# mycorrhiza-inc/fugu

Hardware: AMD Instinct MI355X
Metric: queries/sec + p50 latency, 10M-doc Zipf corpus, 3-term AND, top-100 (higher is better)
Workload: dtype u32+f32; 1 GPU; 3-term AND, BM25 top-100, 10M-doc Zipf s=1.0 corpus per namespace, batch 1024; n_docs=10000000, vocab=1048576, batch=1024, k=100, terms=3, namespaces=1, parallelism=namespace-shard x1

## Files before the change

fugu_amd/csrc/fg_host.h:

```cpp
#pragma once
#include <hip/hip_runtime.h>

#include <algorithm>
#include <atomic>
#include <chrono>
#include <condition_variable>
#include <functional>
#include <cstdint>
#include <map>
#include <memory>
#include <mutex>
#include <string>
#include <thread>
#include <vector>

#include "../../include/fugu.h"
#include "fg_internal.h"
#include "fg_pool.h"
#include "fg_trace.h"

namespace fgh {

int fail(int code, const char* fmt, ...);
int hw_threads(int req);
// ... 312 lines not shown
  std::shared_ptr<DevAllocs> smem;
  std::shared_ptr<ScorePool> spool;
  uint64_t struct_bytes = 0;
  fg::DevIndex d{};
};

struct IndexBounds {
  std::shared_ptr<ScoreBlock> sblock;
  const float* ktop = nullptr;
  const float* tmaxs = nullptr;
  SharedVec<float> wb_text, wb_name;
  float cache_b[512];
  SharedVec<uint32_t> h_alive_b;
  SharedVec<uint64_t> dtab_map;
  uint64_t dtab_bytes = 0;
  SharedVec<uint64_t> dtab8_map;
  uint64_t dtab8_bytes = 0;
  uint64_t device_bytes = 0;
};

inline uint32_t doctab_lead() {
  const char* e = getenv("FUGU_DOCTAB_LEAD");
  return e && *e ? (uint32_t)std::max(0l, atol(e)) : fg::kDocTabLead;
}

inline uint32_t doctab_slot(const IndexBounds& b, uint32_t t) {
  const auto it = std::lower_bound(b.dtab_map.begin(), b.dtab_map.end(), (uint64_t)t << 32);
  return it != b.dtab_map.end() && (uint32_t)(*it >> 32) == t ? (uint32_t)*it + 1u : 0u;
}

inline uint32_t doctab8_lead() {
  const char* e = getenv("FUGU_DOCTAB8_LEAD");
  return e && *e ? (uint32_t)std::max(0l, atol(e)) : fg::kDocTab8Lead;
}

inline uint32_t doctab8_slot(const IndexBounds& b, uint32_t t) {
  const auto it = std::lower_bound(b.dtab8_map.begin(), b.dtab8_map.end(), (uint64_t)t << 32);
  return it != b.dtab8_map.end() && (uint32_t)(*it >> 32) == t ? (uint32_t)*it + 1u : 0u;
}
}

struct fg_index : fgh::IndexStructure, fgh::IndexBounds {
  std::atomic<int> refs{1};
  int dev = 0;
  uint32_t n_dense = 0;
  uint64_t tot[2] = {0, 0};
  uint64_t n_stats = 0;
  float avgdl[2] = {0, 0};
  float cache[512];
  fgh::SharedVec<float> w_text, w_name;
  fgh::SharedVec<float> idf_text, idf_name;
  uint64_t tot_f = 0;
  float avgdl_f = 0.0f, cache_f1 = 0.0f;
  std::vector<uint32_t> df_facet;
  std::vector<float> fscore;
  fgh::SharedVec<uint32_t> h_alive;
  uint32_t n_dead = 0;
  bool same_stats = true;
  double cup[2] = {1, 1}, cdn[2] = {1, 1};
  std::shared_ptr<void> alive_hold;
  std::shared_ptr<const std::vector<float>> kth_floor;
  DevAllocs mem;
  std::shared_ptr<WsPool> pool;
  std::shared_ptr<PinnedPool> pinned;
};

// ... 21 lines not shown
  uint32_t n_prof = 0;
  ~fg_plan() {
    for (hipEvent_t e : pending) (void)hipEventDestroy(e);
    if (pin) {
      (void)hipSetDevice(ix->dev);
      (void)hipStreamSynchronize(up_stream);
    }
    if (ws) {
      if (last_stream_used) {
        (void)hipSetDevice(ix->dev);
        (void)hipStreamSynchronize(last_stream);
      }
      if (pin) ix->pinned->put(pin, pin_n);
      ix->pool->put(ws, ws_got);
    }
    if (!ipc_maps.empty()) {
      (void)hipSetDevice(ix->dev);
      for (void* m : ipc_maps) (void)hipIpcCloseMemHandle(m);
    }
    if (ix) fg_index_release(ix);
    for (fg_index* x : segs) fg_index_release(x);
  }
  bool last_stream_used = false;
  std::vector<uint32_t> h_lo, h_hi;
  std::vector<uint8_t> h_any;
  double part_next = 0.0;
  bool zeroed = false;
  void* pin = nullptr;
  size_t pin_n = 0;
  std::vector<void*> ipc_maps;
  hipStream_t up_stream = hipStreamPerThread;
};


namespace fgh {
inline uint32_t local_term(const fg_index* ix, uint32_t t) {
  if (ix->tmap.empty()) return t;
  const auto it = std::lower_bound(ix->tmap.begin(), ix->tmap.end(), t);
  return it != ix->tmap.end() && *it == t ? (uint32_t)(it - ix->tmap.begin()) : 0xFFFFFFFFu;
}
void term_ratio(const fg_index* ix, uint32_t t, float* rdn, float* rup);
float term_max_now(const fg_index* ix, uint32_t t);
float term_max_scaled(const fg_index* ix, uint32_t t, float rup);
float term_kth_now(const fg_index* ix, uint32_t t, uint32_t k, bool with_floor);

struct Bins { uint32_t lo, hi, shift; };
Bins union_bins(uint32_t lo, uint32_t hi);
int plan_create_multi(fg_index* const* ixs, uint32_t n_segs, const fg_query_batch* q, uint32_t k, fg_plan** out,
                      bool sync, hipStream_t up);
void run_parallel(uint32_t n, const std::function<void(uint32_t)>& f);

hipStream_t build_stream();
bool on_background();
uint32_t bg_grid_cap(int dev);
uint8_t fieldnorm_id(uint64_t n);
void bm25_weights(uint64_t Ns, const uint32_t* df_t, const uint32_t* df_n, uint32_t V, std::vector<float>& wt,
                  std::vector<float>& wn, std::vector<float>& it, std::vector<float>& in);
void set_stats(fg_index* ix, uint64_t Ns, const uint64_t tot2[2], const uint32_t* df_t, const uint32_t* df_n,
               uint64_t tot_f, const uint32_t* df_f, const Weights* wts);
void relate_stats(fg_index* ix);
int dev_upload_bytes(DevAllocs& m, const void* src, size_t n, void** out, uint64_t* bytes);
template <class T>
int dev_upload(DevAllocs& m, const T* src, size_t n, T** out, uint64_t* bytes) {
  return dev_upload_bytes(m, src, n * sizeof(T), reinterpret_cast<void**>(out), bytes);
}
struct UploadBatch {
// ... 20 lines not shown
```

fugu_amd/csrc/fg_internal.h:

```cpp
#pragma once
#include <algorithm>
#include <cstdint>
#include <initializer_list>

#include <hip/hip_runtime.h>

namespace fg {

constexpr uint32_t kBlock = 128;
#ifndef FG_BUCKET
#define FG_BUCKET 4
#endif
constexpr uint32_t kBucketTarget = FG_BUCKET;
constexpr uint32_t kThreads = 256;
#ifndef FG_ITEMS
#define FG_ITEMS 8
#endif
constexpr uint32_t kItems = FG_ITEMS;
constexpr uint32_t kChunk = kThreads * kItems;
constexpr uint32_t kWaveSpan = kChunk / 4;
constexpr uint32_t kMaxTerms = 16;
constexpr uint32_t kMaxK = 1024;
#ifndef FG_FINALCAP
#define FG_FINALCAP 4096
// ... 66 lines not shown
#ifndef FG_DISJ_ROUND
#define FG_DISJ_ROUND 512
#endif
#ifndef FG_DISJ_HBITS
#define FG_DISJ_HBITS 9
#endif
#ifndef FG_DISJ_WAVES
#define FG_DISJ_WAVES 5
#endif
#ifndef FG_DISJ_G
#define FG_DISJ_G 1
#endif
#ifndef FG_DISJ_MAXGROUP
#define FG_DISJ_MAXGROUP 32
#endif
constexpr uint32_t kDisjMaxGroup = FG_DISJ_MAXGROUP;
constexpr uint32_t kDisjMaxPairs = 256;
constexpr uint32_t kNumTopK = 5;
constexpr uint32_t kTopKs[kNumTopK] = {1, 10, 20, 100, 1000};
constexpr uint32_t kNumLadderExtra = 9;
constexpr uint32_t kLadderExtra[kNumLadderExtra] = {2, 3, 5, 13, 25, 50, 125, 250, 500};
constexpr uint32_t kNumLadder = kNumTopK + kNumLadderExtra;
constexpr uint32_t kLadderKs[kNumLadder] = {1, 2, 3, 5, 10, 13, 20, 25, 50, 100, 125, 250, 500, 1000};

constexpr uint32_t kPhraseMaxGroup = 4;
constexpr uint32_t kMaxFacetClauses = 8;
constexpr uint32_t kFmaskChunk = 8192;
constexpr uint32_t kScanMaxGroup = 32;

constexpr uint32_t kModeAnd = 0;
constexpr uint32_t kModeOr = 1;

constexpr uint32_t kQBins = 512;

__host__ __device__ inline uint32_t qm_terms(uint32_t qm) { return qm & 0xFFu; }
__host__ __device__ inline uint32_t qm_must(uint32_t qm) { return (qm >> 8) & 0xFFu; }
__host__ __device__ inline uint32_t qm_not(uint32_t qm) { return (qm >> 16) & 0xFFu; }
__host__ __device__ inline uint32_t qm_pack(uint32_t m, uint32_t nm, uint32_t nx) { return m | (nm << 8) | (nx << 16); }
__host__ __device__ inline uint32_t qm_phrase(uint32_t distinct, uint32_t n) { return distinct | (n << 24); }
__host__ __device__ inline uint32_t qm_phrase_terms(uint32_t qm) { return qm >> 24; }

__host__ __device__ inline uint32_t rank_word(uint32_t d) { return d >> 5; }
__host__ __device__ inline uint32_t rank_pos(uint64_t x, uint32_t d) {
#if defined(__HIP_DEVICE_COMPILE__)
  asm volatile("" : "+v"(d));
#endif
  const uint32_t b = d & 31u;
  if (!((x >> b) & 1ull)) return 0xFFFFFFFFu;
  const uint32_t below = (uint32_t)x & ((1u << b) - 1u);
#if defined(__HIP_DEVICE_COMPILE__)
  return (uint32_t)(x >> 32) + (uint32_t)__popc(below);
#else
  return (uint32_t)(x >> 32) + (uint32_t)__builtin_popcount(below);
#endif
}

__host__ __device__ inline uint32_t srank_block(uint32_t d) { return d >> 10; }
__host__ __device__ inline uint32_t srank_index(uint64_t e, uint32_t d) {
#if defined(__HIP_DEVICE_COMPILE__)
  asm volatile("" : "+v"(d));
#endif
  const uint32_t w = (d >> 5) & 31u;
  const uint32_t below = (uint32_t)e & ((1u << w) - 1u);
#if defined(__HIP_DEVICE_COMPILE__)
  const uint32_t i = (uint32_t)(e >> 32) + (uint32_t)__popc(below);
#else
// ... 176 lines not shown
  if (p1.kind & (kPdDir | kPdWide)) return false;
  if (!probe_uses_bound(ix.n_docs, df, lead_df, tab8_lead)) return false;
  const uint64_t a = (uint64_t)(uintptr_t)(ix.dtab8 + (uint64_t)(tab8 - 1) * ix.dtab8_stride);
  p1.aux_lo = (uint32_t)a;
  p1.kind = (p1.kind & 0xFFFFu) | kPdBound | (uint32_t)((a >> 32) & 0xFFFFu) << 16;
  union { float f; uint32_t u; } c;
  c.f = M;
  lead.aux_lo = c.u;
  return true;
}

struct DevFilters {
  uint32_t n_filters;
  uint32_t n_chunks;
  const uint32_t* q_filter;
  const uint32_t* f_shift;
  const uint64_t* f_woff;
  const float* f_tab;
  const float* f_max;
  const uint32_t* ch_filter;
  const uint32_t* ch_clause;
  const uint32_t* ch_term;
  const uint32_t* ch_start;
  const uint32_t* f_seg;
  uint32_t* fmask;
};

__host__ __device__ inline uint32_t filter_bits(const uint32_t* mask, uint32_t shift, uint32_t d) {
  const uint32_t bit = d << shift;
  return (mask[bit >> 5] >> (bit & 31)) & ((1u << (1u << shift)) - 1u);
}

constexpr uint32_t kMaxPeers = 15;

struct DevPlan {
  uint32_t n_queries;
  uint32_t total_chunks;
  uint32_t k;
  uint32_t n_conj;
  const uint32_t* q_m;
  const uint32_t* q_terms;
  const uint32_t* q_lead_df;
  const uint32_t* work_q;
  const uint32_t* work_c;
  const uint32_t* work_n;
  const uint64_t* cand_off;
  const uint64_t* q_thr0;
  const float* q_ub;
  const ProbeDesc* q_probe;
  const float* q_wt;
  const float* q_wn;
  const float* q_rup;
  const uint32_t* q_hlo;
  const uint32_t* q_hsh;
  uint64_t* thresh;
  uint32_t* hist;
  uint64_t pub_mask;
  uint32_t* cand_cnt;
  uint64_t* cand_keys;
  uint64_t* diag;
  uint32_t feat;
  uint32_t n_single;
  uint32_t n_scan;
  uint32_t n_phrase;
  const uint32_t* q_pterm;
  const uint32_t* q_ppos;
  const DevIndex* segs;
  uint32_t seg_nq;
  uint32_t n_segs;
  const uint32_t* seg_base;
  DevFilters f;
  uint32_t n_peers;
  uint32_t* peer_hist[kMaxPeers];
  uint64_t* peer_thr[kMaxPeers];
};

__host__ __device__ inline uint32_t slot_query(const DevPlan& pl, uint32_t v) {
  return pl.seg_nq ? v % pl.seg_nq : v;
}

constexpr uint32_t kCountItems = 8;
constexpr uint32_t kCountChunk = kThreads * kCountItems;
constexpr uint32_t kCountFacetChunk = kFmaskChunk;
constexpr uint32_t kCountFacetItems = kCountFacetChunk / kThreads;
constexpr uint32_t kCountWordChunk = 2048;
constexpr uint32_t kCountTile = 64;
constexpr uint32_t kCountText = 0, kCountFacet = 1, kCountFill = 2;
struct DevCount {
  uint32_t nq;
  uint32_t q0;
  uint32_t words;
  uint32_t n_count;
  uint32_t n_fchunks, n_items, n_cchunks;
  uint32_t* match;
// ... 169 lines not shown
```

fugu_amd/csrc/fugu.cpp:

```cpp
#include <hip/hip_runtime.h>
#include <sched.h>

#include <algorithm>
#include <atomic>
#include <chrono>
#include <cmath>
#include <condition_variable>
#include <deque>
#include <functional>
#include <cstdarg>
#include <cstdio>
#include <cstring>
#include <map>
#include <memory>
#include <mutex>
#include <string>
#include <thread>
#include <vector>

#include "../../include/fugu.h"
#include "fg_host.h"
#include "fg_internal.h"

namespace {
// ... 963 lines not shown
  return FG_OK;
}

int fg_plan_kernel_ms(fg_plan* p, double* ms_out, uint32_t* n_out) {
  if (!p) return fail(FG_EINVAL, "NULL plan");
  HIPCHK(hipSetDevice(p->ix->dev));
  for (size_t i = 0; i + 2 < p->pending.size(); i += 3) {
    HIPCHK(hipEventSynchronize(p->pending[i + 2]));
    for (int kx = 0; kx < 2; ++kx) {
      float ms = 0;
      HIPCHK(hipEventElapsedTime(&ms, p->pending[i + kx], p->pending[i + kx + 1]));
      p->ms[kx] += ms;
    }
    p->n_prof++;
  }
  for (hipEvent_t e : p->pending) (void)hipEventDestroy(e);
  p->pending.clear();
  if (ms_out) for (int kx = 0; kx < 2; ++kx) ms_out[kx] = p->ms[kx];
  if (n_out) *n_out = p->n_prof;
  p->ms[0] = p->ms[1] = 0;
  p->n_prof = 0;
  return FG_OK;
}

int fg_plan_diag(fg_plan* p, uint64_t* out, size_t n_words, uint32_t* cand_cnt) {
  if (!p) return fail(FG_EINVAL, "NULL plan");
  HIPCHK(hipSetDevice(p->ix->dev));
  HIPCHK(hipStreamSynchronize(p->last_stream));
  if (cand_cnt) HIPCHK(hipMemcpy(cand_cnt, p->d.cand_cnt, 4ull * p->nq, hipMemcpyDeviceToHost));
  if (out && n_words) {
    if (!p->d.diag) return fail(FG_EUNSUPPORTED, "not a diagnostic build (-DFG_DIAG)");
    HIPCHK(hipMemcpy(out, p->d.diag, 8 * std::min(n_words, p->diag_words), hipMemcpyDeviceToHost));
  }
  return FG_OK;
}

int fg_plan_destroy(fg_plan* p) {
  delete p;
  return FG_OK;
}

int fg_plan_link(fg_plan* const* plans, uint32_t n) {
  if (!plans || n == 0) return fail(FG_EINVAL, "bad arguments");
  fg_plan* o = plans[0];
  for (uint32_t i = 0; i < n; ++i) {
    if (!plans[i]) return fail(FG_EINVAL, "NULL plan");
    if (plans[i]->nq != o->nq || plans[i]->k != o->k) return fail(FG_EINVAL, "linked plans differ in batch or k");
    if (plans[i]->ix->dev != o->ix->dev) return fail(FG_EINVAL, "linked plans live on different devices");
    if (plans[i]->n_segs > 1) return fail(FG_EUNSUPPORTED, "a multi-snapshot plan already shares its thresholds");
  }
  const uint32_t nq = o->nq;
  std::vector<uint32_t> lo(nq, 0), sh(nq, 0);
  for (uint32_t q = 0; q < nq; ++q) {
    uint32_t l = 0, h = 0;
    for (uint32_t i = 0; i < n; ++i) {
      l = std::max(l, plans[i]->h_lo[q]);
      h = std::max(h, plans[i]->h_hi[q]);
    }
    const fgh::Bins b = fgh::union_bins(l, h);
    lo[q] = b.lo;
    sh[q] = b.shift;
  }
  HIPCHK(hipSetDevice(o->ix->dev));
  for (uint32_t i = 0; i < n; ++i) {
    fg_plan* p = plans[i];
    if (nq) {
// ... 293 lines not shown
```

fugu_amd/csrc/kernels.hip:

```cpp
#include <hip/hip_runtime.h>

#include "fg_internal.h"

namespace fg {
namespace {

constexpr uint32_t kInvalid = 0xFFFFFFFFu;

#ifdef FG_DIAG
#define FG_STAMP(base, slot, val)                                     \
  do {                                                                \
    if (threadIdx.x == 0 && pl.diag) pl.diag[(base) * kDiagPerWg + (slot)] = (val); \
  } while (0)
#define FG_NOW() __builtin_amdgcn_s_memrealtime()
#else
#define FG_STAMP(base, slot, val) do { } while (0)
#define FG_NOW() 0ull
#endif

__device__ inline uint32_t lane_id() { return threadIdx.x & 63; }

typedef const __attribute__((address_space(4))) DevIndex ConstDevIndex;
__device__ inline DevIndex seg_index(const DevPlan& pl, uint32_t s) {
#if defined(__HIP_DEVICE_COMPILE__)
// ... 95 lines not shown
__device__ inline float term_bound(const DevIndex& ix, uint32_t meta, uint32_t toff, uint32_t dir_off, uint32_t d) {
  return toff != 0xFFFFFFFFu ? ix.tmax[toff + (d >> kDisjTileShift)] : ix.bmax[dir_off + (d >> (meta & 0xFFu))];
}

__device__ inline bool term_has_doc(const DevIndex& ix, uint32_t meta, uint64_t base, uint32_t dir_off, uint32_t d) {
  const uint32_t slot = meta_slot(meta);
  if (slot) return (rank_word_of(ix, slot, d) >> (d & 31u)) & 1ull;
  const uint32_t* __restrict__ dir = ix.dir + dir_off;
  const uint32_t b = d >> (meta & 0xFFu);
  uint32_t lo = dir[b], hi = dir[b + 1];
  const uint32_t* __restrict__ di = ix.doc + base;
  while (lo < hi) {
    const uint32_t mid = (lo + hi) >> 1;
    if (di[mid] < d) lo = mid + 1; else hi = mid;
  }
  return lo < dir[b + 1] && di[lo] == d;
}

__device__ inline uint32_t posting_pos(const DevIndex& ix, uint32_t t, uint32_t d) {
  const uint32_t meta = ix.tmeta[t], slot = meta_slot(meta);
  if (slot) return rank_pos(rank_word_of(ix, slot, d), d);
  const uint32_t* __restrict__ dir = ix.dir + ix.dir_off[t];
  const uint32_t b = d >> (meta & 0xFFu);
  uint32_t lo = dir[b], hi = dir[b + 1];
  const uint32_t* __restrict__ di = ix.doc + ix.off[t];
  while (lo < hi) {
    const uint32_t mid = (lo + hi) >> 1;
    if (di[mid] < d) lo = mid + 1; else hi = mid;
  }
  return lo < dir[b + 1] && di[lo] == d ? lo : kInvalid;
}


__device__ inline uint32_t qbin(uint64_t key, uint32_t lo, uint32_t sh) {
  const uint32_t bits = (uint32_t)(key >> 32);
  if (bits < lo) return kQBins;
  return min((bits - lo) >> sh, kQBins - 1);
}

__device__ inline uint32_t block_exclusive_scan(uint32_t v, uint32_t* scratch ) {
  const uint32_t lane = lane_id(), w = wave_id();
  uint32_t incl = v;
#pragma unroll
  for (int o = 1; o < 64; o <<= 1) {
    const uint32_t y = (uint32_t)__shfl_up((int)incl, o, 64);
    if (lane >= (uint32_t)o) incl += y;
  }
  if (lane == 63) scratch[w] = incl;
  __syncthreads();
  uint32_t base = 0;
#pragma unroll
  for (uint32_t i = 0; i < kThreads / 64; ++i) base += i < w ? scratch[i] : 0u;
  __syncthreads();
  return base + incl - v;
}

__device__ uint64_t hist_threshold(const uint32_t* gh, uint32_t K, uint32_t lo, uint32_t sh, uint32_t* scratch) {
  static_assert(kQBins == 2 * kThreads, "two bins per thread");
  const uint32_t tid = threadIdx.x;
  const uint32_t b0 = kQBins - 1 - 2 * tid, b1 = b0 - 1;
  const uint32_t v0 = __hip_atomic_load(gh + b0, __ATOMIC_RELAXED, __HIP_MEMORY_SCOPE_AGENT);
  const uint32_t v1 = __hip_atomic_load(gh + b1, __ATOMIC_RELAXED, __HIP_MEMORY_SCOPE_AGENT);
  if (tid == 0) scratch[5] = kQBins;
  const uint32_t before = block_exclusive_scan(v0 + v1, scratch);
  if (before < K && before + v0 >= K) scratch[5] = b0;
  else if (before + v0 < K && before + v0 + v1 >= K) scratch[5] = b1;
  __syncthreads();
  const uint32_t b = scratch[5];
  __syncthreads();
  return b < kQBins ? (uint64_t)(lo + (b << sh)) << 32 : 0ull;
}

constexpr uint64_t kScoreOnly = 0xFFFFFFFF00000000ull;

__device__ inline void peer_thr_max(const DevPlan& pl, uint32_t ql, uint64_t key) {
  for (uint32_t i = 0; i < pl.n_peers; ++i)
    atomicMax(reinterpret_cast<unsigned long long*>(pl.peer_thr[i] + ql), (unsigned long long)(key & kScoreOnly));
}

__device__ inline void hist_add(uint32_t* lh, uint32_t* gh, const DevPlan& pl, uint32_t ql) {
  for (uint32_t i = 0; i < pl.n_peers; ++i)
    for (uint32_t b = threadIdx.x; b < kQBins; b += kThreads)
      if (const uint32_t c = lh[b]) atomicAdd(pl.peer_hist[i] + (size_t)ql * kQBins + b, c);
  for (uint32_t b = threadIdx.x; b < kQBins; b += kThreads) {
    const uint32_t c = lh[b];
    if (c) {
      atomicAdd(&gh[b], c);
      lh[b] = 0;
    }
  }
}

__device__ inline void wave_append(bool keep, uint64_t key, uint64_t* list, uint32_t* count, uint32_t cap) {
  const uint32_t lane = lane_id();
  const unsigned long long bal = __ballot(keep);
  const uint32_t nw = (uint32_t)__popcll(bal);
  if (!nw) return;
  uint32_t base = 0;
  if (lane == 0) base = atomicAdd(count, nw);
  base = (uint32_t)__shfl((int)base, 0, 64);
  const uint32_t at = base + (uint32_t)__popcll(bal & ((1ull << lane) - 1ull));
  if (keep && at < cap) list[at] = key;
}

template <uint32_t Bits = kHistBits, class Each>
__device__ uint64_t select_kth(uint32_t K, uint32_t* hist, uint32_t* scratch, Each each) {
  constexpr uint32_t kBins = 1u << Bits;
  const uint32_t tid = threadIdx.x, lane = lane_id(), wv = wave_id();
  uint64_t kor = 0, kand = ~0ull;
  each([&](uint64_t k) { kor |= k; kand &= k; });
#pragma unroll
  for (int o = 32; o > 0; o >>= 1) {
    kor |= (uint64_t)__shfl_xor((long long)kor, o, 64);
    kand &= (uint64_t)__shfl_xor((long long)kand, o, 64);
  }
  uint64_t* red = reinterpret_cast<uint64_t*>(hist);
// ... 576 lines not shown
    }
    __syncthreads();
    uint32_t n = sh.n_buf;
    uint64_t tp2 = FG_NOW();
    (void)tp2;
    if (defer) {
      const uint32_t nd = min(sh.n_dq, kDeferCap);
      if (nd >= kDeferFlush || (cc + 1 == nc && nd > 0)) {
        if (n > kTrunc) {
          local_T = truncate_topk(sh, n, K);
          if (local_T > thr_k) thr_k = local_T;
        }
        flush_deferred<kF>(ix, sh, probes, terms, qwt, qwn, m, thr_k, nd);
        __syncthreads();
        n = sh.n_buf;
        if (tid == 0) sh.n_dq = 0;
      }
    }
    if (n > kTrunc || (cc + 1 == nc && n > K)) {
      local_T = truncate_topk(sh, n, K);
      if (local_T > thr_k) thr_k = local_T;
    }
    uint64_t tp3 = FG_NOW();
    (void)tp3;
#ifdef FG_DIAG
    t_probe += tp1 - tp0; t_keys += tp2 - tp1; t_sel += tp3 - tp2; n_app += n;
#endif
    if (tid == 0) {
      if (local_T > sh.thr) sh.thr = local_T;
      pend = atomicMax(gthr, (unsigned long long)(local_T & pl.pub_mask));
    }
  }
  if (tid == 0 && pend > sh.thr) sh.thr = pend;
  if (tid == 0) peer_thr_max(pl, ql, sh.thr);
  __syncthreads();

  const uint32_t total = flush_candidates(pl, q, sh.buf, sh.n_buf, sh.thr, sh.scratch);
  (void)total;
  {
    static_assert((1u << kConjHistBits) >= kQBins, "LDS bins");
    const uint32_t n = min(sh.n_buf, kBuf);
    for (uint32_t b = tid; b < kQBins; b += kThreads) sh.hist[b] = 0;
    __syncthreads();
    for (uint32_t i = tid; i < n; i += kThreads) {
      const uint32_t b = qbin(sh.buf[i], h_lo, h_sh);
      if (b < kQBins) atomicAdd(&sh.hist[b], 1u);
    }
    __syncthreads();
    hist_add(sh.hist, gh, pl, ql);
  }
  FG_STAMP(w, 0, t_start);
  FG_STAMP(w, 1, t_probe);
  FG_STAMP(w, 2, t_keys);
  FG_STAMP(w, 3, t_sel);
  FG_STAMP(w, 4, FG_NOW());
  FG_STAMP(w, 5, n_app);
  FG_STAMP(w, 6, ((uint64_t)nc << 40) | ((uint64_t)m << 32) | q);
  FG_STAMP(w, 7, total);
#ifdef FG_DIAG
  __syncthreads();
  for (uint32_t i = 0; i < 8; ++i) FG_STAMP(w, 8 + i, sh.dgc[i]);
#endif
}

constexpr uint32_t kTileShift = kDisjTileShift;
constexpr uint32_t kTile = 1u << kTileShift;
constexpr uint32_t kRound = FG_DISJ_ROUND;
constexpr uint32_t kBufD = kTrunc + kRound;
constexpr uint32_t kPairs = kRound;
constexpr uint32_t kQCap = 2 * kRound;
constexpr uint32_t kDisjHistBits = FG_DISJ_HBITS;
constexpr uint32_t kMaxTiles = kDisjMaxGroup;
constexpr uint32_t kMaxSeg = kDisjMaxPairs;
static_assert(kMaxSeg <= 2 * kThreads, "k_disj segment list: two (tile, clause) pairs per thread");
static_assert(kMaxTiles <= 255 && kMaxTerms <= 16, "seg_info packs (tile << 4) | clause; cand (tile << 8) | clause");

template <bool kQt>
struct DisjQt {
  float c_wt[kMaxTerms], c_wn[kMaxTerms];
  float cache[256];
};
template <>
struct DisjQt<false> {};
// ... 2231 lines not shown
```

fugu_amd/csrc/plan.cpp:

```cpp
#include <chrono>
#include <cstdio>
#include <cstdlib>
#include <cstring>

#include "fg_host.h"

using fgh::fail;

fgh::Bins fgh::union_bins(uint32_t lo, uint32_t hi) {
  hi = std::max(hi, lo);
  uint32_t sh = 0;
  while (sh < 31 && ((uint64_t)(hi - lo) >> sh) >= fg::kQBins - 1) ++sh;
  return Bins{lo, hi, sh};
}

namespace {

void radix_sort_hi32(std::vector<uint64_t>& a, std::vector<uint64_t>& tmp) {
  tmp.resize(a.size());
  for (int sh = 32; sh < 64; sh += 11) {
    uint32_t cnt[2049] = {0};
    for (uint64_t x : a) cnt[((x >> sh) & 2047u) + 1]++;
    for (int d = 0; d < 2048; ++d) cnt[d + 1] += cnt[d];
    for (uint64_t x : a) tmp[cnt[(x >> sh) & 2047u]++] = x;
// ... 166 lines not shown
      const uint32_t t = c[i];
      if (t >= ix->n_fterms || ix->df_facet[t] == 0) continue;
      f_lo[f] = std::min(f_lo[f], ix->ffirst[t]);
      f_hi[f] = std::max(f_hi[f], ix->flast[t]);
      const uint64_t df = ix->foff[t + 1] - ix->foff[t];
      for (uint64_t st = 0; st < df; st += fg::kFmaskChunk) {
        h.ch_f.push_back(f);
        h.ch_c.push_back(i);
        h.ch_t.push_back(t);
        h.ch_s.push_back((uint32_t)st);
      }
    }
  }

  const uint32_t gpq_batch =
      fg::kGroupsPerQuery * std::min<uint32_t>(fg::kDisjSmallSpread, std::max<uint32_t>(1, 256 / std::max(nq_size, 1u)));
  const uint32_t gpq = std::max<uint32_t>(1, gpq_batch / n_segs);
  const uint32_t conj_gpq = fg::kConjGroupsPerQuery, conj_maxg = fg::kMaxGroup;
  const uint32_t cdiv = n_segs <= 1 ? 1u : n_segs;
  h.ngroup.assign(nq, 0);
  for (auto* v : {&h.q_hlo, &h.q_hhi}) v->assign(nq, 0x3F800000u);
  h.q_hsh.assign(nq, 31);
  auto present = [&](uint32_t t) { return t < ix->n_terms && ix->off[t + 1] > ix->off[t]; };
  float cm[fg::kMaxTerms];
  auto set_clause = [&](uint32_t i, uint32_t j, uint32_t t) {
    const size_t x = (size_t)i * fg::kMaxTerms + j;
    h.q_wt[x] = ix->w_text[t];
    h.q_wn[x] = ix->w_name[t];
    float rdn, rup;
    fgh::term_ratio(ix, t, &rdn, &rup);
    h.q_rup[x] = rup;
    cm[j] = fgh::term_max_scaled(ix, t, rup);
  };
  auto set_bins = [&](uint32_t i, float ub) {
    const float lo = h.thr0[i] ? fg::key_score(h.thr0[i]) : ub / 256.0f;
    uint32_t lb, hb;
    std::memcpy(&lb, &lo, 4);
    std::memcpy(&hb, &ub, 4);
    const fgh::Bins b = fgh::union_bins(std::max<uint32_t>(lb, 1), hb);
    h.q_hlo[i] = b.lo;
    h.q_hhi[i] = b.hi;
    h.q_hsh[i] = b.shift;
  };
  for (uint32_t i = 0; i < nq; ++i) {
    const uint32_t b = q->q_off[i], e = q->q_off[i + 1];
    if (e < b) return fail(FG_EINVAL, "q_off not monotone at query %u", i);
    const uint32_t m = e - b;
    if (m > fg::kMaxTerms) return fail(FG_EUNSUPPORTED, "query %u has %u terms (> %u)", i, m, fg::kMaxTerms);
    if (q->phrase_len) {
      int phrase = 0;
      if (int rc = plan_phrase(ix, q, i, nq_size, n_segs, h, &phrase)) return rc;
      if (phrase) continue;
    }
    if (q_nomatch[i]) continue;
    const uint32_t flt = h.q_filter[i];
    const float fmx = flt == 0xFFFFFFFFu ? 0.0f : h.f_max[flt];
    if (m == 0) {
      h.q_m[i] = 0;
      const uint64_t dlo = flt == 0xFFFFFFFFu ? 0 : f_lo[flt], dhi = flt == 0xFFFFFFFFu ? N - 1 : f_hi[flt];
      const uint32_t tlo = (uint32_t)(dlo >> fg::kDisjTileShift), thi = (uint32_t)(dhi >> fg::kDisjTileShift);
      const uint32_t nt = thi - tlo + 1;
      const uint32_t G = std::min<uint32_t>(fg::kScanMaxGroup,
                                            std::max<uint32_t>(1, (nt + gpq - 1) / gpq));
      const uint32_t ng = (nt + G - 1) / G;
      h.ngroup[i] = ng;
      for (uint32_t g = 0; g < ng; ++g) h.scan.push_back(WItem{(double)g, i, tlo + g * G, std::min(G, nt - g * G)});
      continue;
    }
// ... 64 lines not shown
    for (uint32_t j = 0; j < nm; ++j) qt[j] = tc[j].term;
    for (uint32_t j = 0; j < nx; ++j) qt[nm + j] = tx[j];
    for (uint32_t j = 0; j < ns; ++j) qt[nm + nx + j] = ts_[j];
    const uint32_t mt = nm + nx + ns;
    for (uint32_t j = 0; j < mt; ++j) set_clause(i, j, qt[j]);
    h.q_m[i] = fg::qm_pack(mt, nm, nx);
    {
      float acc = 0.0f;
      for (uint32_t j = mt; j-- > 1;) {
        if (j < nm || j >= nm + nx) acc += cm[j];
        h.q_ub[(size_t)i * fg::kMaxTerms + j] = acc;
      }
      const size_t row = (size_t)i * fg::kMaxTerms;
      const uint64_t lead_df = ix->off[qt[0] + 1] - ix->off[qt[0]];
      for (uint32_t j = 0; j < mt; ++j) {
        const uint32_t t = qt[j];
        const uint32_t tab = j && !qtime && !ix->dtab_map.empty() ? fgh::doctab_slot(*ix, t) : 0u;
        const fg::ProbeTerm pt{ix->off[t], ix->off[t + 1], ix->tmeta[t], ix->dir_off[t], tab};
        h.q_probe[row + j] =
            fg::probe_desc(ix->d, pt, j == 0, qtime, j + 1 < mt ? h.q_ub[row + j + 1] : 0.0f, lead_df, tab_lead);
      }
      if (!qtime && !ix->dtab8_map.empty() && mt >= 3 && nm == mt && flt == 0xFFFFFFFFu)
        fg::probe_desc_bound(ix->d, h.q_probe[row], h.q_probe[row + 1], fgh::doctab8_slot(*ix, qt[1]), ix->tmaxs[qt[1]],
                             true, qtime, ix->off[qt[1] + 1] - ix->off[qt[1]], lead_df, tab8_lead);
    }
    if (mt == 1 && flt == 0xFFFFFFFFu) {
      const float v = fgh::term_kth_now(ix, qt[0], k, true);
      if (v > 0.0f) h.thr0[i] = fg::make_key(v, 0xFFFFFFFFu);
    }
    {
      float ub = fmx + cm[0];
      for (uint32_t j = 1; j < mt; ++j)
        if (j < nm || j >= nm + nx) ub += cm[j];
      set_bins(i, ub);
    }
    const uint64_t df0 = ix->off[qt[0] + 1] - ix->off[qt[0]];
    h.lead[i] = (uint32_t)df0;
    const uint32_t nch = (uint32_t)((df0 + fg::kChunk - 1) / fg::kChunk);
    if (h.citems.size() + nch > 0x7FFFFFFFull)
      return fail(FG_EUNSUPPORTED, "batch too large (%zu work items)", h.citems.size());
    const uint32_t per_q =
        std::max<uint32_t>(1, std::min<uint32_t>(64, std::max<uint32_t>(conj_gpq, 1024 / std::max(nq_size, 1u))) / cdiv);
    const uint32_t G = std::min<uint32_t>(conj_maxg, std::max<uint32_t>(1, (nch + per_q - 1) / per_q));
    const uint32_t ng = (nch + G - 1) / G;
    h.ngroup[i] = ng;
    for (uint32_t g = 0; g < ng; ++g)
      h.citems.push_back(WItem{(g + 0.5) / ng, i, g * G, std::min(G, nch - g * G)});
  }
  return FG_OK;
}

struct Pieces {
  uint32_t S = 1, nq1 = 0, P = 1;
  uint32_t count() const { return S * P; }
  uint32_t begin(uint32_t r) const { return (uint32_t)((uint64_t)nq1 * r / P); }
  uint32_t slot(uint32_t pc) const { return (pc / P) * nq1 + begin(pc % P); }
};

int plan_pieces(fg_index* const* ixs, uint32_t S, const fg_query_batch* q, uint32_t k, std::vector<PlanTables>& hs,
                PlanTables& J, Pieces& pc) {
  if (!ixs || !q || S == 0 || S > FG_MAX_SEGMENTS) return fail(FG_EINVAL, "bad arguments");
  for (uint32_t s = 0; s < S; ++s) {
    if (!ixs[s]) return fail(FG_EINVAL, "NULL snapshot");
    if (ixs[s]->dev != ixs[0]->dev) return fail(FG_EINVAL, "the snapshots of one plan live on different devices");
  }
  const uint32_t nq1 = q->n_queries;
  if ((uint64_t)S * nq1 > 0x7FFFFFFFull) return fail(FG_EUNSUPPORTED, "batch too large (%u x %u query slots)", S, nq1);
// ... 333 lines not shown
  if (!p->diag_words) d.diag = nullptr;
  p->zero_region = base + s_in;
  p->zero_bytes = s_zero;
  HIPCHK(hipMemcpyAsync(base, staging, s_up, hipMemcpyHostToDevice, up));
  p->up_stream = up;
  p->zeroed = s_up > s_in;
  if (sync || !pin.p) {
    HIPCHK(hipStreamSynchronize(up));
  } else {
    p->pin = pin.p;
    p->pin_n = pin.n;
    pin.p = nullptr;
  }
  return FG_OK;
}

void fill_view(fg_plan* p, fg_index* const* ixs, PlanTables& t, const WorkList& w) {
  const uint32_t S = p->n_segs, nq = p->nq, nq1 = p->nq_batch;
  p->d.n_queries = nq;
  p->d.total_chunks = (uint32_t)w.n_main;
  p->d.n_conj = (uint32_t)w.n_conj;
  p->d.n_scan = (uint32_t)w.n_scan;
  p->d.n_phrase = (uint32_t)w.n_phrase;
  p->d.n_single = (uint32_t)w.n_single;
  p->d.k = p->k;
  p->d.seg_nq = S > 1 ? nq1 : 0;
  p->d.n_segs = S;
  p->d.feat = 0;
  for (uint32_t x = 0; x < S; ++x)
    if (!ixs[x]->same_stats) p->d.feat = 4u;
  for (uint32_t x = 0; x < S && p->d.feat; ++x)
    p->d.feat |= (ixs[x]->d.tfn_name ? 1u : 0u) | (ixs[x]->d.n_esc ? 2u : 0u);
  p->d.pub_mask = S > 1 ? 0xFFFFFFFF00000000ull : ~0ull;
  p->h_any.assign(nq1, 0);
  for (uint32_t v = 0; v < nq; ++v)
    if (t.ngroup[v]) p->h_any[v % nq1] = 1;
  p->h_lo.swap(t.q_hlo);
  p->h_hi.swap(t.q_hhi);
  p->d.f.n_filters = t.nf;
  p->d.f.n_chunks = (uint32_t)t.ch_f.size();
}

}

int fgh::plan_create_multi(fg_index* const* ixs, uint32_t S, const fg_query_batch* q, uint32_t k, fg_plan** out,
                           bool sync, hipStream_t up) {
  if (!out) return fail(FG_EINVAL, "bad arguments");
  static const bool ptrace = getenv("FUGU_SHARD_TRACE") != nullptr;
  auto pnow = [] { return std::chrono::duration<double, std::milli>(std::chrono::steady_clock::now().time_since_epoch()).count(); };
  double pt[5] = {ptrace ? pnow() : 0.0, 0, 0, 0, 0};
  static thread_local std::vector<PlanTables> hs_tl;
  static thread_local PlanTables J_tl;
  static thread_local WorkList w_tl;
  Pieces pc;
  if (int rc = plan_pieces(ixs, S, q, k, hs_tl, J_tl, pc)) return rc;
  if (ptrace) pt[1] = pnow();
  PlanTables& t = join_pieces(pc, hs_tl, J_tl);
  if (ptrace) pt[2] = pnow();
  const uint32_t nq1 = pc.nq1, nq = S * nq1;
  WorkList& w = w_tl;
  if (int rc = order_items(t, nq, k, w)) return rc;
  if (ptrace) pt[3] = pnow();
  auto p = std::make_unique<fg_plan>();
  p->nq = nq;
  p->nq_batch = nq1;
  p->n_segs = S;
// ... 24 lines not shown
```

fugu_amd/native.py:

```python
from __future__ import annotations

import ctypes as C
import os
from dataclasses import dataclass

import numpy as np

import torch

_HERE = os.path.dirname(os.path.abspath(__file__))
LIB_PATH = os.environ.get("FUGU_LIB") or os.path.join(_HERE, "libfugu.so")

FG_OK = 0
FG_EINVAL = -1
FG_ENODEV = -2
FG_EOOM = -3
FG_EHIP = -4
FG_EUNSUPPORTED = -5
FG_MAX_TERMS = 16
FG_MAX_FACET_CLAUSES = 8
FG_MAX_K = 1024
FG_TERM_MISSING = 0xFFFFFFFF
FG_MAX_COUNT_TERMS = 1 << 20
FG_MAX_COUNT_CELLS = 1 << 25
# ... 129 lines not shown
_sig("fg_index_rescore", C.c_int, _p, C.POINTER(GlobalStats), _u8p, C.POINTER(_p))
_sig("fg_index_rescore_many", C.c_int, C.POINTER(_p), C.c_uint32, C.POINTER(GlobalStats), C.POINTER(_u8p),
     C.POINTER(_p))
_sig("fg_index_retain", C.c_int, _p)
_sig("fg_thread_background", C.c_int, C.c_int)
_sig("fg_index_release", C.c_int, _p)
_sig("fg_index_stats_get", C.c_int, _p, C.POINTER(IndexStats))
_sig("fg_index_doctab_get", C.c_int, _p, _u32p, _u64p)
if hasattr(_lib, "fg_index_doctab8_get"):
    _sig("fg_index_doctab8_get", C.c_int, _p, _u32p, _u64p)
_sig("fg_index_df", C.c_uint64, _p, C.c_int, C.c_uint32)
_sig("fg_index_bm25", C.c_int, _p, C.c_uint32, _f32p, _f32p, _f32p)
_sig("fg_plan_create", C.c_int, _p, C.POINTER(QueryBatch), C.c_uint32, C.POINTER(_p))
_sig("fg_plan_create_multi", C.c_int, C.POINTER(_p), C.c_uint32, C.POINTER(QueryBatch), C.c_uint32, C.POINTER(_p))
_sig("fg_plan_execute_merged", C.c_int, _p, _p, _p, _p, _p, _p)
_sig("fg_index_term_kth", C.c_int, _p, C.c_uint32, _f32p)
_sig("fg_index_term_ladder", C.c_int, _p, _f32p)
_sig("fg_kth_floor_combine", C.c_int, C.c_uint32, C.c_uint32, C.POINTER(_f32p), _f32p)
_sig("fg_index_set_kth_floor", C.c_int, _p, _f32p, C.c_uint32)
_sig("fg_plan_execute", C.c_int, _p, _p, _p, _p, _p)
_sig("fg_plan_results", C.c_int, _p, _f32p, _u32p, _u32p)
_sig("fg_plan_hist_span", C.c_int, _p, _u32p, _u32p)
_sig("fg_plan_set_hist_span", C.c_int, _p, _u32p, _u32p)
_sig("fg_plan_execute_part", C.c_int, _p, _p, C.c_double, C.c_double, _p, _p, _p, _p)
_sig("fg_plan_hist_copy", C.c_int, _p, _p, _p, C.c_int)
_sig("fg_plan_set_peers", C.c_int, _p, C.POINTER(_p), C.c_uint32)
_sig("fg_plan_ipc_export", C.c_int, _p, C.POINTER(PlanIpc))
_sig("fg_plan_set_ipc_peers", C.c_int, _p, C.POINTER(PlanIpc), C.c_uint32)
_sig("fg_plan_reset", C.c_int, _p, _p)
_sig("fg_plan_info_get", C.c_int, _p, C.POINTER(PlanInfo))
_sig("fg_plan_profile", C.c_int, _p, C.c_int)
_sig("fg_plan_kernel_ms", C.c_int, _p, _f64p, _u32p)
_sig("fg_plan_diag", C.c_int, _p, _u64p, C.c_size_t, _u32p)
_sig("fg_plan_destroy", C.c_int, _p)
_sig("fg_search_batch", C.c_int, _p, C.POINTER(QueryBatch), C.c_uint32, _f32p, _u32p, _u32p)
_sig("fg_search_sharded", C.c_int, _p, C.POINTER(_p), C.c_uint32, C.POINTER(QueryBatch), C.c_uint32, _f32p, _u32p,
     _u32p, _u32p)
_sig("fg_merge_shards", C.c_int, C.c_uint32, C.c_uint32, C.c_uint32, _p, _p, _p, _p, _p, _p, _p, _p)
_sig("fg_bytes_model", C.c_int, _p, C.POINTER(QueryBatch), C.c_uint32, _f64p)
_sig("fg_bytes_model_gpu", C.c_int, _p, C.POINTER(QueryBatch), C.c_uint32, _f64p)
_sig("fg_model_batch", C.c_int, _p, C.POINTER(QueryBatch), C.c_uint32, _f32p, _f64p, C.POINTER(ModelOut))
_sig("fg_count_batch", C.c_int, C.POINTER(_p), C.c_uint32, C.POINTER(QueryBatch), _u32p, C.c_uint32, _u64p, _u64p)
_sig("fg_count_trace", C.c_int, C.c_int, _f64p, _u32p)
_sig("fg_abi_version", C.c_int)
if _lib.fg_abi_version() != ABI_VERSION:
    raise ImportError(f"{LIB_PATH} has ABI {_lib.fg_abi_version()}, this binding follows {ABI_VERSION}: rebuild")


class FuguError(RuntimeError):
    def __init__(self, code: int, msg: str):
        super().__init__(f"libfugu error {code}: {msg}")
        self.code = code


class Unsupported(FuguError):
    """FG_EUNSUPPORTED: the query is outside the device subset (host CPU path)."""


def _check(rc: int):
    if rc != FG_OK:
        msg = (_lib.fg_last_error() or b"").decode(errors="replace")
        if rc == FG_EUNSUPPORTED:
            raise Unsupported(rc, msg)
        raise FuguError(rc, msg)


# ... 439 lines not shown
    def ipc_export(self) -> bytes:
        x = PlanIpc()
        _check(_lib.fg_plan_ipc_export(self._h, C.byref(x)))
        return bytes(x)

    def set_ipc_peers(self, blobs):
        arr = (PlanIpc * max(len(blobs), 1))()
        for i, b in enumerate(blobs):
            if len(b) != C.sizeof(PlanIpc):
                raise ValueError(f"peer {i}: {len(b)} bytes, expected {C.sizeof(PlanIpc)}")
            C.memmove(C.byref(arr, i * C.sizeof(PlanIpc)), b, len(b))
        _check(_lib.fg_plan_set_ipc_peers(self._h, arr, len(blobs)))

    def reset(self, stream: int | None = None):
        _check(_lib.fg_plan_reset(self._h, stream))

    def results(self):
        nq, k = self.n_queries, self.k
        score = np.zeros(nq * k, np.float32)
        doc = np.zeros(nq * k, np.uint32)
        n = np.zeros(nq, np.uint32)
        _check(_lib.fg_plan_results(self._h, _ptr(score, _f32p), _ptr(doc, _u32p), _ptr(n, _u32p)))
        return score.reshape(nq, k), doc.reshape(nq, k), n

    def profile(self, enable: bool = True):
        _check(_lib.fg_plan_profile(self._h, 1 if enable else 0))

    def kernel_ms(self):
        ms = np.zeros(2, np.float64)
        n = C.c_uint32(0)
        _check(_lib.fg_plan_kernel_ms(self._h, _ptr(ms, _f64p), C.byref(n)))
        return ms, n.value

    def candidate_counts(self):
        cnt = np.zeros(self.n_queries, np.uint32)
        _check(_lib.fg_plan_diag(self._h, None, 0, _ptr(cnt, _u32p)))
        return cnt

    def diag(self):
        info = self.info()
        n = DIAG_PER_WG * (info.total_chunks + self.n_queries)
        out = np.zeros(n, np.uint64)
        _check(_lib.fg_plan_diag(self._h, _ptr(out, _u64p), n, None))
        w = out.reshape(-1, DIAG_PER_WG)
        return w[: info.total_chunks], w[info.total_chunks:]

    def close(self):
        if self._h:
            _lib.fg_plan_destroy(self._h)
            self._h = None

    def __del__(self):
        try:
            self.close()
        except Exception:
            pass


def kth_floor_combine(ladders) -> np.ndarray:
    ls = [np.ascontiguousarray(x, np.float32) for x in ladders]
    if not ls:
        raise ValueError("no ladders")
    V = ls[0].shape[0]
    for x in ls:
        if x.shape != (V, len(LADDER_KS)):
            raise ValueError(f"ladder shape {x.shape}, expected ({V}, {len(LADDER_KS)})")
# ... 53 lines not shown
```

Before: 1.137 million queries/s.

## Derive conjunctive threshold from global histogram during merge before flushing candidates

In the conjunctive kernel, the local score histogram is now merged into the global histogram before candidate flushing, using the atomicAdd return values to find the k-th bin edge. That edge then raises the block threshold and the published global threshold. The intent is to prune more candidates at flush time and cut candidate writes and later top-k work. It also adds a configurable histogram lower bound divisor and a host API for seeding initial thresholds, at the cost of extra block scans and synchronisation per chunk.

```diff
diff --git a/fugu_amd/csrc/fg_host.h b/fugu_amd/csrc/fg_host.h
--- a/fugu_amd/csrc/fg_host.h
+++ b/fugu_amd/csrc/fg_host.h
@@ -368,6 +368,17 @@
 inline uint32_t doctab8_lead() {
   const char* e = getenv("FUGU_DOCTAB8_LEAD");
   return e && *e ? (uint32_t)std::max(0l, atol(e)) : fg::kDocTab8Lead;
+}
+
+inline bool conj_hist_thr() {
+  const char* e = getenv("FUGU_CONJ_HIST_THR");
+  return !(e && *e) || atol(e) != 0;
+}
+
+inline float hist_lo_div() {
+  const char* e = getenv("FUGU_HIST_LO_DIV");
+  const double v = e && *e ? atof(e) : 0.0;
+  return v >= 1.0 ? (float)v : 256.0f;
 }
 
 inline uint32_t doctab8_slot(const IndexBounds& b, uint32_t t) {
@@ -455,6 +466,7 @@
   hipStream_t up_stream = hipStreamPerThread;
 };
 
+extern "C" int fg_plan_seed_thr0(fg_plan* p, const float* score, uint32_t n);
 
 namespace fgh {
 inline uint32_t local_term(const fg_index* ix, uint32_t t) {
diff --git a/fugu_amd/csrc/fg_internal.h b/fugu_amd/csrc/fg_internal.h
--- a/fugu_amd/csrc/fg_internal.h
+++ b/fugu_amd/csrc/fg_internal.h
@@ -122,6 +122,22 @@
 constexpr uint32_t kModeOr = 1;
 
 constexpr uint32_t kQBins = 512;
+
+__host__ __device__ inline uint32_t qbin(uint64_t key, uint32_t lo, uint32_t sh) {
+  const uint32_t bits = (uint32_t)(key >> 32);
+  if (bits < lo) return kQBins;
+  const uint32_t b = (bits - lo) >> sh;
+  return b < kQBins - 1 ? b : kQBins - 1;
+}
+
+__host__ __device__ inline uint64_t hist_kth_edge(const uint32_t* c, uint32_t n, uint32_t first, uint32_t before,
+                                                  uint32_t K, uint32_t lo, uint32_t sh) {
+  for (uint32_t i = 0; i < n; ++i) {
+    if (before < K && before + c[i] >= K) return (uint64_t)(lo + ((first - i) << sh)) << 32;
+    before += c[i];
+  }
+  return 0ull;
+}
 
 __host__ __device__ inline uint32_t qm_terms(uint32_t qm) { return qm & 0xFFu; }
 __host__ __device__ inline uint32_t qm_must(uint32_t qm) { return (qm >> 8) & 0xFFu; }
@@ -364,6 +380,7 @@
 }
 
 constexpr uint32_t kMaxPeers = 15;
+constexpr uint32_t kOptConjHistThr = 1u;
 
 struct DevPlan {
   uint32_t n_queries;
@@ -392,6 +409,7 @@
   uint64_t* cand_keys;
   uint64_t* diag;
   uint32_t feat;
+  uint32_t opts;
   uint32_t n_single;
   uint32_t n_scan;
   uint32_t n_phrase;
diff --git a/fugu_amd/csrc/fugu.cpp b/fugu_amd/csrc/fugu.cpp
--- a/fugu_amd/csrc/fugu.cpp
+++ b/fugu_amd/csrc/fugu.cpp
@@ -1019,6 +1019,20 @@
     if (!p->d.diag) return fail(FG_EUNSUPPORTED, "not a diagnostic build (-DFG_DIAG)");
     HIPCHK(hipMemcpy(out, p->d.diag, 8 * std::min(n_words, p->diag_words), hipMemcpyDeviceToHost));
   }
+  return FG_OK;
+}
+
+int fg_plan_seed_thr0(fg_plan* p, const float* score, uint32_t n) {
+  if (!p || !score || n != p->nq_batch) return fail(FG_EINVAL, "bad arguments");
+  std::vector<uint64_t> t((size_t)p->nq);
+  for (uint32_t v = 0; v < p->nq; ++v) {
+    const float s = score[v % p->nq_batch];
+    t[v] = s > 0.0f ? fg::make_key(s, 0xFFFFFFFFu) : 0ull;
+  }
+  HIPCHK(hipSetDevice(p->ix->dev));
+  if (p->pin) HIPCHK(hipStreamSynchronize(p->up_stream));
+  if (p->last_stream_used) HIPCHK(hipStreamSynchronize(p->last_stream));
+  if (p->nq) HIPCHK(hipMemcpy(const_cast<uint64_t*>(p->d.q_thr0), t.data(), 8ull * p->nq, hipMemcpyHostToDevice));
   return FG_OK;
 }
 
diff --git a/fugu_amd/csrc/kernels.hip b/fugu_amd/csrc/kernels.hip
--- a/fugu_amd/csrc/kernels.hip
+++ b/fugu_amd/csrc/kernels.hip
@@ -151,12 +151,6 @@
 }
 
 
-__device__ inline uint32_t qbin(uint64_t key, uint32_t lo, uint32_t sh) {
-  const uint32_t bits = (uint32_t)(key >> 32);
-  if (bits < lo) return kQBins;
-  return min((bits - lo) >> sh, kQBins - 1);
-}
-
 __device__ inline uint32_t block_exclusive_scan(uint32_t v, uint32_t* scratch ) {
   const uint32_t lane = lane_id(), w = wave_id();
   uint32_t incl = v;
@@ -174,20 +168,26 @@
   return base + incl - v;
 }
 
-__device__ uint64_t hist_threshold(const uint32_t* gh, uint32_t K, uint32_t lo, uint32_t sh, uint32_t* scratch) {
+__device__ inline uint64_t block_kth_edge(uint32_t v0, uint32_t v1, uint32_t K, uint32_t lo, uint32_t sh,
+                                          uint32_t* scratch) {
   static_assert(kQBins == 2 * kThreads, "two bins per thread");
   const uint32_t tid = threadIdx.x;
-  const uint32_t b0 = kQBins - 1 - 2 * tid, b1 = b0 - 1;
+  if (tid == 0) scratch[5] = 0;
+  const uint32_t before = block_exclusive_scan(v0 + v1, scratch);
+  const uint32_t c[2] = {v0, v1};
+  const uint64_t e = hist_kth_edge(c, 2, kQBins - 1 - 2 * tid, before, K, lo, sh);
+  if (e) scratch[5] = (uint32_t)(e >> 32);
+  __syncthreads();
+  const uint32_t bits = scratch[5];
+  __syncthreads();
+  return (uint64_t)bits << 32;
+}
+
+__device__ uint64_t hist_threshold(const uint32_t* gh, uint32_t K, uint32_t lo, uint32_t sh, uint32_t* scratch) {
+  const uint32_t b0 = kQBins - 1 - 2 * threadIdx.x, b1 = b0 - 1;
   const uint32_t v0 = __hip_atomic_load(gh + b0, __ATOMIC_RELAXED, __HIP_MEMORY_SCOPE_AGENT);
   const uint32_t v1 = __hip_atomic_load(gh + b1, __ATOMIC_RELAXED, __HIP_MEMORY_SCOPE_AGENT);
-  if (tid == 0) scratch[5] = kQBins;
-  const uint32_t before = block_exclusive_scan(v0 + v1, scratch);
-  if (before < K && before + v0 >= K) scratch[5] = b0;
-  else if (before + v0 < K && before + v0 + v1 >= K) scratch[5] = b1;
-  __syncthreads();
-  const uint32_t b = scratch[5];
-  __syncthreads();
-  return b < kQBins ? (uint64_t)(lo + (b << sh)) << 32 : 0ull;
+  return block_kth_edge(v0, v1, K, lo, sh, scratch);
 }
 
 constexpr uint64_t kScoreOnly = 0xFFFFFFFF00000000ull;
@@ -197,10 +197,24 @@
     atomicMax(reinterpret_cast<unsigned long long*>(pl.peer_thr[i] + ql), (unsigned long long)(key & kScoreOnly));
 }
 
-__device__ inline void hist_add(uint32_t* lh, uint32_t* gh, const DevPlan& pl, uint32_t ql) {
+__device__ inline void hist_add_peers(const uint32_t* lh, const DevPlan& pl, uint32_t ql) {
   for (uint32_t i = 0; i < pl.n_peers; ++i)
     for (uint32_t b = threadIdx.x; b < kQBins; b += kThreads)
       if (const uint32_t c = lh[b]) atomicAdd(pl.peer_hist[i] + (size_t)ql * kQBins + b, c);
+}
+
+__device__ inline uint64_t hist_add_kth(const uint32_t* lh, uint32_t* gh, const DevPlan& pl, uint32_t ql, uint32_t cut,
+                                        uint32_t K, uint32_t lo, uint32_t sh, uint32_t* scratch) {
+  hist_add_peers(lh, pl, ql);
+  const uint32_t b0 = kQBins - 1 - 2 * threadIdx.x, b1 = b0 - 1;
+  const uint32_t c0 = lh[b0], c1 = lh[b1];
+  const uint32_t v0 = (c0 || b0 >= cut) ? atomicAdd(&gh[b0], c0) + c0 : 0u;
+  const uint32_t v1 = (c1 || b1 >= cut) ? atomicAdd(&gh[b1], c1) + c1 : 0u;
+  return block_kth_edge(v0, v1, K, lo, sh, scratch);
+}
+
+__device__ inline void hist_add(uint32_t* lh, uint32_t* gh, const DevPlan& pl, uint32_t ql) {
+  hist_add_peers(lh, pl, ql);
   for (uint32_t b = threadIdx.x; b < kQBins; b += kThreads) {
     const uint32_t c = lh[b];
     if (c) {
@@ -843,11 +857,6 @@
     }
   }
   if (tid == 0 && pend > sh.thr) sh.thr = pend;
-  if (tid == 0) peer_thr_max(pl, ql, sh.thr);
-  __syncthreads();
-
-  const uint32_t total = flush_candidates(pl, q, sh.buf, sh.n_buf, sh.thr, sh.scratch);
-  (void)total;
   {
     static_assert((1u << kConjHistBits) >= kQBins, "LDS bins");
     const uint32_t n = min(sh.n_buf, kBuf);
@@ -858,8 +867,23 @@
       if (b < kQBins) atomicAdd(&sh.hist[b], 1u);
     }
     __syncthreads();
-    hist_add(sh.hist, gh, pl, ql);
-  }
+    if (!kSingle && (pl.opts & kOptConjHistThr)) {
+      const uint64_t cur = sh.thr;
+      const uint32_t cb = qbin(cur, h_lo, h_sh);
+      const uint64_t edge = hist_add_kth(sh.hist, gh, pl, ql, cur && cb < kQBins ? cb : 0u, K, h_lo, h_sh, sh.scratch);
+      if (tid == 0 && edge > cur) {
+        sh.thr = edge;
+        atomicMax(gthr, (unsigned long long)(edge & pl.pub_mask));
+      }
+    } else {
+      hist_add(sh.hist, gh, pl, ql);
+    }
+  }
+  if (tid == 0) peer_thr_max(pl, ql, sh.thr);
+  __syncthreads();
+
+  const uint32_t total = flush_candidates(pl, q, sh.buf, sh.n_buf, sh.thr, sh.scratch);
+  (void)total;
   FG_STAMP(w, 0, t_start);
   FG_STAMP(w, 1, t_probe);
   FG_STAMP(w, 2, t_keys);
diff --git a/fugu_amd/csrc/plan.cpp b/fugu_amd/csrc/plan.cpp
--- a/fugu_amd/csrc/plan.cpp
+++ b/fugu_amd/csrc/plan.cpp
@@ -222,8 +222,9 @@
     h.q_rup[x] = rup;
     cm[j] = fgh::term_max_scaled(ix, t, rup);
   };
-  auto set_bins = [&](uint32_t i, float ub) {
-    const float lo = h.thr0[i] ? fg::key_score(h.thr0[i]) : ub / 256.0f;
+  const float conj_lo_div = fgh::hist_lo_div();
+  auto set_bins = [&](uint32_t i, float ub, float div = 256.0f) {
+    const float lo = h.thr0[i] ? fg::key_score(h.thr0[i]) : ub / div;
     uint32_t lb, hb;
     std::memcpy(&lb, &lo, 4);
     std::memcpy(&hb, &ub, 4);
@@ -354,7 +355,7 @@
       float ub = fmx + cm[0];
       for (uint32_t j = 1; j < mt; ++j)
         if (j < nm || j >= nm + nx) ub += cm[j];
-      set_bins(i, ub);
+      set_bins(i, ub, conj_lo_div);
     }
     const uint64_t df0 = ix->off[qt[0] + 1] - ix->off[qt[0]];
     h.lead[i] = (uint32_t)df0;
@@ -754,6 +755,7 @@
   for (uint32_t x = 0; x < S && p->d.feat; ++x)
     p->d.feat |= (ixs[x]->d.tfn_name ? 1u : 0u) | (ixs[x]->d.n_esc ? 2u : 0u);
   p->d.pub_mask = S > 1 ? 0xFFFFFFFF00000000ull : ~0ull;
+  p->d.opts = fgh::conj_hist_thr() ? fg::kOptConjHistThr : 0u;
   p->h_any.assign(nq1, 0);
   for (uint32_t v = 0; v < nq; ++v)
     if (t.ngroup[v]) p->h_any[v % nq1] = 1;
diff --git a/fugu_amd/native.py b/fugu_amd/native.py
--- a/fugu_amd/native.py
+++ b/fugu_amd/native.py
@@ -185,6 +185,8 @@
 _sig("fg_plan_profile", C.c_int, _p, C.c_int)
 _sig("fg_plan_kernel_ms", C.c_int, _p, _f64p, _u32p)
 _sig("fg_plan_diag", C.c_int, _p, _u64p, C.c_size_t, _u32p)
+if hasattr(_lib, "fg_plan_seed_thr0"):
+    _sig("fg_plan_seed_thr0", C.c_int, _p, _f32p, C.c_uint32)
 _sig("fg_plan_destroy", C.c_int, _p)
 _sig("fg_search_batch", C.c_int, _p, C.POINTER(QueryBatch), C.c_uint32, _f32p, _u32p, _u32p)
 _sig("fg_search_sharded", C.c_int, _p, C.POINTER(_p), C.c_uint32, C.POINTER(QueryBatch), C.c_uint32, _f32p, _u32p,
@@ -690,6 +692,12 @@
         _check(_lib.fg_plan_kernel_ms(self._h, _ptr(ms, _f64p), C.byref(n)))
         return ms, n.value
 
+    def seed_thresholds(self, score):
+        s = np.ascontiguousarray(score, np.float32)
+        if s.shape != (self.n_batch,):
+            raise ValueError(f"scores of {s.shape}, expected ({self.n_batch},)")
+        _check(_lib.fg_plan_seed_thr0(self._h, _ptr(s, _f32p), self.n_batch))
+
     def candidate_counts(self):
         cnt = np.zeros(self.n_queries, np.uint32)
         _check(_lib.fg_plan_diag(self._h, None, 0, _ptr(cnt, _u32p)))
```

Result: faster. 1.198 million queries/s (median of 6 runs) (+5.4%).
